# DHDev0/Stochastic-muzero

Hardware: AMD Instinct MI355X
Metric: MCTS simulations/sec (whole node), CartPole MLP 4096 envs × 50 sims (higher is better)
Workload: dtype f32 (tree values, heads) + f64 (pUCT scores, root priors) + i32 (counts)

## Files before the change

### stochastic-muzero_amd/csrc/smz_mlp_device.hpp

```cpp
#pragma once
#include <hip/hip_runtime.h>
#include <math.h>
#include <stdint.h>

#include "../../include/smz.h"

namespace smz_mlp {

constexpr int kWave = 64;
enum { M_DYN_IN, M_ADY_IN, M_DYN_MID, M_ADY_MID, M_DYN_OUT, M_ADY_OUT, M_PRE_IN, M_APR_IN, M_PRE_MID, M_APR_MID,
       M_PRE_OUT, M_APR_OUT, M_REP_IN, M_REP_MID, M_REP_OUT, M_COUNT };

__host__ __device__ inline int up4(int x) { return (x + 3) & ~3; }

typedef float v2f __attribute__((ext_vector_type(2)));
__device__ inline v2f pk_fma(float wx, float wy, float ax, float ay, v2f c) {
    v2f w = {wx, wy}, a = {ax, ay};
    return __builtin_elementwise_fma(w, a, c);
}
template <int U, int R, bool SAME = false>
__device__ inline void dense(const float *const (&W)[R], const float *const (&bias)[R], const float *const (&act)[R], int K4,
                             const int (&OP)[R], int lane, float (&acc)[R][U]) {
    const float4 *a4[R], *w4[R];
    v2f acc2[R][U];
// ... 515 lines not shown

constexpr int kRows = 1;

__host__ __device__ inline int row_scratch_floats(const smz_mlp_desc &d) {
    const int kin = up4(d.S + d.A) > up4(d.obs) ? up4(d.S + d.A) : up4(d.obs);
    return kin + up4(d.H) + up4(d.S);
}
__host__ __device__ inline int scratch_floats(const smz_mlp_desc &d) { return kRows * row_scratch_floats(d); }

template <int U, int R, bool SAME = false, bool CP = false>
__device__ inline void recurrent_rows(const float *lds, const smz_mlp_desc &d, float *scratch, const float *const (&xin)[R],
                                      const bool (&dyn)[R], const bool (&live)[R], float *const (&dst_hidden)[R],
                                      float *const (&dst_policy)[R], float (&reward)[R], float (&value)[R]) {
    const int S = d.S, A = d.A, K4in = up4(S + A), K4h = up4(d.H), K4s = up4(S);
    const int lane = threadIdx.x & (kWave - 1);
    const int rs = row_scratch_floats(d), kin = rs - K4h - K4s;
    float *tA[R], *hbuf[R];
    MatOff m1[R], m1m[R], m3[R], m3m[R];
#pragma unroll
    for (int r = 0; r < R; r++) {
        tA[r] = scratch + r * rs + kin;
        hbuf[r] = tA[r] + K4h;
        m1[r] = pick<CP>(d, dyn[r], M_DYN_IN, M_ADY_IN);   m1m[r] = pick<CP>(d, dyn[r], M_DYN_MID, M_ADY_MID);
        m3[r] = pick<CP>(d, dyn[r], M_PRE_IN, M_APR_IN);   m3m[r] = pick<CP>(d, dyn[r], M_PRE_MID, M_APR_MID);
        for (int k = lane; k < K4s; k += kWave) hbuf[r][k] = 0.f;
    }
    trunk<U, R, SAME>(lds, d, m1, m1m, xin, K4in, tA, lane);
    float acc[R][U];
    constexpr bool PAIRED = SMZ_PAIR_TAILS && U == 1 && R == 2;
    const bool halves = PAIRED && SAME && SMZ_DENSE_HALVES && S <= 32 && !dyn[0] && !dyn[1];
    if (halves) {
        if constexpr (PAIRED && SAME) {
            const MatOff m = pick<CP>(d, false, M_DYN_OUT, M_ADY_OUT);
            acc[0][0] = dense_halves(lds + m.w, lds + m.b, tA[0], tA[1], K4h, m.op, lane);
            acc[1][0] = 0.f;
        }
    } else {
        const float *W[R], *Bv[R], *Ac[R];
        int op[R];
#pragma unroll
        for (int r = 0; r < R; r++) {
            const MatOff m = pick<CP>(d, dyn[r], M_DYN_OUT, M_ADY_OUT);
            W[r] = lds + m.w; Bv[r] = lds + m.b; Ac[r] = tA[r]; op[r] = m.op;
        }
        dense<U, R, SAME>(W, Bv, Ac, K4h, op, lane, acc);
    }
    float pair_rnum = 0.f, pair_rden = 0.f;
    bool pair_reward = false;
    if constexpr (PAIRED) {
        if (S <= 32) {
            reward[0] = reward[1] = 0.f;
            if (halves) scale_pair<true>(acc[0][0], 0.f, S, lane, hbuf[0], hbuf[1], live[0] ? dst_hidden[0] : nullptr,
                                         live[1] ? dst_hidden[1] : nullptr);
            else if (!dyn[0] && !dyn[1]) scale_pair(acc[0][0], acc[1][0], S, lane, hbuf[0], hbuf[1], live[0] ? dst_hidden[0] : nullptr,
                                               live[1] ? dst_hidden[1] : nullptr);
            else if (SMZ_ONE_DECODE) {
                dynamics_tail_pair<true>(acc[0][0], acc[1][0], dyn[0], dyn[1], S, lane, hbuf[0], hbuf[1], live[0] ? dst_hidden[0] : nullptr,
                                         live[1] ? dst_hidden[1] : nullptr, reward[0], reward[1], &pair_rnum, &pair_rden);
                pair_reward = true;
            } else dynamics_tail_pair(acc[0][0], acc[1][0], dyn[0], dyn[1], S, lane, hbuf[0], hbuf[1], live[0] ? dst_hidden[0] : nullptr,
                                      live[1] ? dst_hidden[1] : nullptr, reward[0], reward[1]);
        } else {
#pragma unroll
            for (int r = 0; r < R; r++) {
                reward[r] = 0.f;
                if (dyn[r]) reward[r] = decode_scale_lanes<U>(acc[r], S, lane, hbuf[r], live[r] ? dst_hidden[r] : nullptr);
                else scale_lanes<U>(acc[r], 0, S, lane, hbuf[r], live[r] ? dst_hidden[r] : nullptr);
            }
        }
    } else {
#pragma unroll
    for (int r = 0; r < R; r++) {
        reward[r] = 0.f;
        if (dyn[r]) {
            reward[r] = decode_scale_lanes<U>(acc[r], S, lane, hbuf[r], live[r] ? dst_hidden[r] : nullptr);
        } else {
            scale_lanes<U>(acc[r], 0, S, lane, hbuf[r], live[r] ? dst_hidden[r] : nullptr);
        }
    }
    }
    lds_sync();
    {
        const float *Hc[R];
#pragma unroll
        for (int r = 0; r < R; r++) Hc[r] = hbuf[r];
        trunk<U, R, SAME>(lds, d, m3, m3m, Hc, K4s, tA, lane);
        const float *W[R], *Bv[R], *Ac[R];
        int op[R];
#pragma unroll
        for (int r = 0; r < R; r++) {
            const MatOff m = pick<CP>(d, dyn[r], M_PRE_OUT, M_APR_OUT);
            W[r] = lds + m.w; Bv[r] = lds + m.b; Ac[r] = tA[r]; op[r] = m.op;
        }
        dense<U, R, SAME>(W, Bv, Ac, K4h, op, lane, acc);
    }
    if constexpr (PAIRED) {
        if (S <= 32 && A <= 32 && pair_reward) {
            float r0, r1;
            softmax_decode_pair<true>(acc[0][0], acc[1][0], A, S, lane, live[0] ? dst_policy[0] : nullptr,
                                      live[1] ? dst_policy[1] : nullptr, value[0], value[1], pair_rnum, pair_rden, &r0, &r1);
            reward[0] = dyn[0] ? r0 : 0.f;
            reward[1] = dyn[1] ? r1 : 0.f;
        } else if (S <= 32 && A <= 32) {
            softmax_decode_pair(acc[0][0], acc[1][0], A, S, lane, live[0] ? dst_policy[0] : nullptr, live[1] ? dst_policy[1] : nullptr,
                                value[0], value[1]);
        } else {
#pragma unroll
            for (int r = 0; r < R; r++) value[r] = softmax_decode_lanes<U>(acc[r], A, S, lane, live[r] ? dst_policy[r] : nullptr);
        }
    } else {
#pragma unroll
    for (int r = 0; r < R; r++) {
        value[r] = softmax_decode_lanes<U>(acc[r], A, S, lane, live[r] ? dst_policy[r] : nullptr);
    }
    }
    lds_sync();
}

template <int U, bool CP = false>
__device__ inline void initial_row(const float *lds, const smz_mlp_desc &d, const float *rep, const smz_mlp_desc &drep,
                                   float *scratch, const float *obs_row, float *dst_hidden0, float *dst_hidden1,
                                   float *dst_policy) {
    const int S = d.S, A = d.A, K4o = up4(d.obs), K4h = up4(d.H), K4s = up4(S);
    const int lane = threadIdx.x & (kWave - 1);
    const int rs = row_scratch_floats(d), kin = rs - K4h - K4s;
    float *xbuf = scratch;
    float *tA[1] = {scratch + kin};
    float *hbuf = tA[0] + K4h;
    for (int k = lane; k < K4o; k += kWave) xbuf[k] = (k < d.obs) ? obs_row[k] : 0.f;
    for (int k = lane; k < K4s; k += kWave) hbuf[k] = 0.f;
    lds_sync();
    const MatOff mi[1] = {pick(drep, true, M_REP_IN, M_REP_IN)}, mm[1] = {pick(drep, true, M_REP_MID, M_REP_MID)};
    const float *xi[1] = {xbuf};
    trunk<U, 1>(rep, drep, mi, mm, xi, K4o, tA, lane);
    float acc[1][U];
    {
        const float *W[1] = {rep + drep.off[M_REP_OUT]}, *Bv[1] = {rep + drep.off[M_COUNT + M_REP_OUT]}, *Ac[1] = {tA[0]};
        dense<U, 1>(W, Bv, Ac, K4h, d.OP, lane, acc);
    }
    scale_lanes<U>(acc[0], 0, S, lane, hbuf, dst_hidden0, dst_hidden1);
    lds_sync();
    const MatOff pi[1] = {pick<CP>(d, true, M_PRE_IN, M_PRE_IN)}, pm[1] = {pick<CP>(d, true, M_PRE_MID, M_PRE_MID)};
    const float *hi[1] = {hbuf};
    trunk<U, 1>(lds, d, pi, pm, hi, K4s, tA, lane);
    {
        const MatOff po = pick<CP>(d, true, M_PRE_OUT, M_PRE_OUT);
        const float *W[1] = {lds + po.w}, *Bv[1] = {lds + po.b}, *Ac[1] = {tA[0]};
        dense<U, 1>(W, Bv, Ac, K4h, po.op, lane, acc);
    }
    softmax_lanes<U>(acc[0], A, lane, dst_policy);
    lds_sync();
}

__host__ __device__ inline int rep_floats(const smz_mlp_desc &d) { return d.off[M_COUNT] - d.off[M_REP_IN]; }
__host__ __device__ inline smz_mlp_desc lds_desc_without_rep(const smz_mlp_desc &d) {
    smz_mlp_desc l = d;
    const int rs = rep_floats(d);
    for (int m = 0; m < M_COUNT; m++) l.off[M_COUNT + m] = d.off[M_COUNT + m] - rs;
    l.total_floats = d.total_floats - rs;
    return l;
}
__device__ inline void stage_weights_without_rep(float *lds, const float *weights, const smz_mlp_desc &d) {
    constexpr int UB = 8;
    const int n_mat = d.off[M_REP_IN], n_bias = d.total_floats - d.off[M_COUNT], rs = rep_floats(d);
    for (int pass = 0; pass < 2; pass++) {
        const float *src = pass ? weights + d.off[M_COUNT] : weights;
        float *dst = pass ? lds + d.off[M_COUNT] - rs : lds;
        const int cnt = pass ? n_bias : n_mat;
        for (int i0 = threadIdx.x * 4; i0 < cnt; i0 += blockDim.x * 4 * UB) {
            float4 v[UB];
#pragma unroll
            for (int u = 0; u < UB; u++) { const int i = i0 + u * blockDim.x * 4; v[u] = *reinterpret_cast<const float4 *>(src + (i < cnt ? i : i0)); }
#pragma unroll
            for (int u = 0; u < UB; u++) { const int i = i0 + u * blockDim.x * 4; if (i < cnt) *reinterpret_cast<float4 *>(dst + i) = v[u]; }
        }
    }
    __syncthreads();
}

__host__ __device__ inline int compact_matrix_floats(const smz_mlp_desc &d) { return mat_off<true>(d, M_REP_IN); }
__host__ __device__ inline int compact_total_floats(const smz_mlp_desc &d) { return compact_matrix_floats(d) + (d.total_floats - d.off[M_COUNT]); }
__device__ inline smz_mlp_desc lds_desc_compact(const smz_mlp_desc &d) {
    smz_mlp_desc l = d;
    l.off[M_COUNT] = compact_matrix_floats(d);
    l.total_floats = compact_total_floats(d);
    return l;
}
__device__ inline void stage_weights_compact(float *lds, const float *weights, const smz_mlp_desc &d) {
    const int kin = up4(d.S + d.A), kmid = d.L > 0 ? up4(d.H) : 0, kh = up4(d.H), ks = up4(d.S);
    const int K[M_REP_IN] = {kin, kin, kmid, kmid, kh, kh, ks, ks, kmid, kmid, kh, kh};
    int dst = 0;
#pragma unroll
    for (int m = 0; m < M_REP_IN; m++) {
        const int op = mat_op<true>(d, m), groups = K[m] >> 2, per = op;
        const float4 *src = reinterpret_cast<const float4 *>(weights + d.off[m]);
        float4 *out = reinterpret_cast<float4 *>(lds + dst);
        for (int i = threadIdx.x; i < groups * per; i += blockDim.x) {
            const int g = i / per, o = i - g * per;
            out[i] = src[g * d.OP + o];
        }
        dst += K[m] * op;
    }
    const int n_bias = d.total_floats - d.off[M_COUNT];
    for (int i = threadIdx.x * 4; i < n_bias; i += blockDim.x * 4)
        *reinterpret_cast<float4 *>(lds + dst + i) = *reinterpret_cast<const float4 *>(weights + d.off[M_COUNT] + i);
    __syncthreads();
}

__device__ inline void stage_recurrent_weights(float *lds, const float *weights, const smz_mlp_desc &d) {
    const int ranges[4] = {0, d.off[M_REP_IN], d.off[M_COUNT], d.off[M_COUNT + M_REP_IN] - d.off[M_COUNT]};
    stage_weights(lds, weights, ranges, 2);
}
__device__ inline void stage_all_weights(float *lds, const float *weights, const smz_mlp_desc &d) {
    const int ranges[2] = {0, d.total_floats};
    stage_weights(lds, weights, ranges, 1);
}
__device__ inline void stage_initial_weights(float *lds, const float *weights, const smz_mlp_desc &d) {
    const int ranges[10] = {d.off[M_REP_IN], d.off[M_COUNT] - d.off[M_REP_IN],
                            d.off[M_PRE_IN], d.off[M_APR_IN] - d.off[M_PRE_IN],
                            d.off[M_PRE_MID], d.off[M_APR_MID] - d.off[M_PRE_MID],
                            d.off[M_PRE_OUT], d.off[M_APR_OUT] - d.off[M_PRE_OUT],
                            d.off[M_COUNT], d.total_floats - d.off[M_COUNT]};
    stage_weights(lds, weights, ranges, 5);
}

}
```

### stochastic-muzero_amd/csrc/smz_search_mlp.hpp

```cpp
#pragma once
#include "smz_common.hpp"
#include "smz_handle.hpp"

namespace {

extern __shared__ float4 smz_search_lds4[];

#ifndef SMZ_BPS_HBM
#define SMZ_BPS_HBM 1
#endif
#ifndef SMZ_SELECT_BLOCKS
#define SMZ_SELECT_BLOCKS 1
#endif
#ifndef SMZ_EARLY_ROWS
#define SMZ_EARLY_ROWS 1
#endif
#ifndef SMZ_PAIR_A4
#define SMZ_PAIR_A4 1
#endif
#ifndef SMZ_SELECT_TWO_PASSES
#define SMZ_SELECT_TWO_PASSES 1
#endif
#ifndef SMZ_LEAF_FIRST
#define SMZ_LEAF_FIRST 1
#endif
#ifndef SMZ_EARLY_STAGE
#define SMZ_EARLY_STAGE 1
#endif
#ifndef SMZ_SELECT_MASKS
#define SMZ_SELECT_MASKS 1
#endif
#ifdef SMZ_BPS_PROBE
#define SMZ_PROBE_DECL unsigned long long pb_t0 = 0, pb_acc[7] = {0, 0, 0, 0, 0, 0, 0};
#define SMZ_PROBE_START pb_t0 = __builtin_amdgcn_s_memtime();
#define SMZ_PROBE_AT(i) { const unsigned long long pb_t1 = __builtin_amdgcn_s_memtime(); pb_acc[i] += pb_t1 - pb_t0; pb_t0 = pb_t1; }
#if SMZ_BPS_PROBE + 0 == 2
#define SMZ_PROBE(i)
#define SMZ_PROBE_B(i) SMZ_PROBE_AT(i)
#else
#define SMZ_PROBE(i) SMZ_PROBE_AT(i)
#define SMZ_PROBE_B(i)
#endif
#define SMZ_PROBE_FLUSH(stats) if ((stats) && lane == 0) { for (int pb_i = 0; pb_i < 7; pb_i++) atomicAdd(&(stats)[8 + pb_i], pb_acc[pb_i]); }
#else
#define SMZ_PROBE_DECL
#define SMZ_PROBE_START
#define SMZ_PROBE(i)
#define SMZ_PROBE_B(i)
#define SMZ_PROBE_FLUSH(stats)
#endif

struct MegaLds {
    int pbc_off, wave_off, per_wave;
    int x_off, pv_off, rng_off, out_off, sel_off, sel_n;
    int sel_on;
    int trees_off, tree_words;
};
__host__ __device__ inline MegaLds mega_lds(const smz_mlp_desc &d, const Params &P, int tpw, bool tlds = false, int waves = 8) {
    MegaLds m;
    m.pbc_off = r4(tlds ? smz_mlp::compact_total_floats(d) : d.total_floats - smz_mlp::rep_floats(d));
    m.wave_off = m.pbc_off + r4(2 * 2 * (P.sims + 2));
    m.x_off = r4(2 * smz_mlp::row_scratch_floats(d));
    m.pv_off = m.x_off + tpw * smz_mlp::up4(P.S + P.A);
    m.rng_off = m.pv_off + tpw * P.P * 4;
    m.out_off = m.rng_off + r4(tpw * kRngStride);
    m.sel_off = m.out_off + r4(tpw * (P.A + 2));
    m.sel_n = (P.sims + 2 + 1) & ~1;
    bool sel = tlds;
    if (!tlds && SMZ_BPS_HBM && P.A == 2 && P.K == 2 && tpw == 2 && P.sims <= 126) {
        const int per = m.sel_off + r4(tpw * m.sel_n);
        sel = ((size_t)m.wave_off + (size_t)waves * per) * sizeof(float) <= (size_t)160 * 1024;
    }
    m.sel_on = sel ? 1 : 0;
    m.per_wave = m.sel_off + (sel ? r4(tpw * m.sel_n) : 0);
    m.tree_words = r4(P.rb_words + P.sims * 6 * P.K + (P.K == 2 ? 2 * P.sims : 0));
    m.trees_off = m.wave_off + waves * m.per_wave;
    return m;
}

constexpr int kFastTpw = 2, kFastS = 31, kFastH = 64, kFastL = 0;
template <int MAXA, int KS, int U, bool INSTR, bool AEX, bool MSK = true, bool PHX = false, bool TLDS = false>
__global__ void __launch_bounds__(SMZ_SEARCH_THREADS) k_search_mlp(Params Pin, smz_mlp_desc d, const float *weights, const float *obs,
                                                    int train, ActOut act, EnvStep env) {
    Params P = Pin;
    P.tree0 = 0;
    if (AEX) { P.A = MAXA; P.tpw = kFastTpw; d.A = MAXA; d.S = kFastS; d.H = kFastH; d.L = kFastL; d.OP = smz_mlp::kWave; P.S = kFastS; }
    if (AEX) P.philox = PHX ? 1 : 0;
    if (KS > 0) P.K = KS;
    fix_layout(P, AEX, KS > 0);
    if (AEX) P.hs = (kFastS + 15) & ~15;
    float *lds = reinterpret_cast<float *>(smz_search_lds4);
    static_assert(!TLDS || (AEX && KS > 0), "LDS-resident trees: the specialised instantiations only");
    const smz_mlp_desc dl = TLDS ? smz_mlp::lds_desc_compact(d) : smz_mlp::lds_desc_without_rep(d);
    if (TLDS) smz_mlp::stage_weights_compact(lds, weights, d);
    else smz_mlp::stage_weights_without_rep(lds, weights, d);
    const int lane = threadIdx.x & (kWave - 1), wave = threadIdx.x / kWave, waves = blockDim.x / kWave;
    const int A = P.A, S = P.S, tpw = P.tpw;
    const MegaLds ml = mega_lds(d, P, tpw, TLDS, waves);
    uint32_t *const nodes_global = P.nodes;
    const int gl_eb_words = P.eb_words;
    if (TLDS) {
        uint32_t *nodes_lds = reinterpret_cast<uint32_t *>(lds + ml.trees_off);
        for (int i = threadIdx.x; i < waves * tpw * ml.tree_words; i += blockDim.x) nodes_lds[i] = 0u;
        P.nodes = nodes_lds;
        P.tree0 = blockIdx.x * waves * tpw;
        P.eb_words = 6 * KS;
        P.tree_words = ml.tree_words;
    }
    constexpr bool THR = AEX && KS == 2, YV = THR && TLDS;
    if (THR) {
        P.thr_off = TLDS ? P.rb_words + P.sims * 6 * KS : P.rb_words + 12;
        P.thr_stride = TLDS ? 2 : P.eb_words;
        P.ry_off = (YV && MAXA <= 8 && P.rp_off + 3 * A <= P.rb_words) ? P.rp_off + 2 * A : -1;
    }
    double *pbc_lds = reinterpret_cast<double *>(lds + ml.pbc_off);
    const int n_pbc = P.sims + 2;
    for (int i = threadIdx.x; i < n_pbc; i += blockDim.x) {
        pbc_lds[i] = P.pbc_sqrt[i];
        pbc_lds[n_pbc + i] = i > 0 ? 1.0 / (double)i : 0.0;
    }
    const int slot = A + 2;
    const int K4in = smz_mlp::up4(S + A);
    float *scratch = lds + ml.wave_off + wave * ml.per_wave;
    float *xall = scratch + ml.x_off;
    uint4 *pvals = reinterpret_cast<uint4 *>(scratch + ml.pv_off);
    uint32_t *rng_tile = reinterpret_cast<uint32_t *>(scratch + ml.rng_off);
    float *outs = scratch + ml.out_off;
    __syncthreads();

    const int tree0 = (blockIdx.x * waves + wave) * tpw;
    const int tree = tree0 + lane;
    const bool valid = lane < tpw && tree < P.B && (!MSK || tree_active(P, tree));
    if (MSK && __ballot(valid) == 0ull) {
        if (env.state && lane < tpw && tree < P.B) cartpole_env_step(env, tree, P.B, act.action, act.policy, act.child_visits, act.root_value);
        return;
    }

    for (int t = 0; t < tpw; t++) {
        const int row = tree0 + t;
        if (row >= P.B) break;
        if (MSK && !__shfl((int)valid, t)) continue;
        smz_mlp::initial_row<U, TLDS>(lds, dl, weights, d, scratch, obs + (size_t)row * d.obs, P.hidden + (size_t)row * P.N * P.hs,
                                      nullptr, outs + t * slot);
    }
    constexpr bool PHC = !AEX || PHX;
    int packed = wave_stage_rng<PHC>(P, tree, valid, rng_tile);
    RngT<PHC> rng;
    rng.bind(P, tree, valid);
    TreeHdr h = {0, 0, 0.f, 0.f, 0, 0.f, 0, 0};
    if (valid) {
        rng.load(P.mt + (size_t)tree * kMtN, packed, rng_tile + lane * kRngStride, kRngStage);
        root_init_tree<MAXA>(P, tree, rng, outs + lane * slot, nullptr, train != 0);
        h = P.hdr[tree];
        packed = rng.pack();
    }
    unsigned n_dec = 0, n_chance = 0, n_children = 0, n_desc = 0;
    const int vmask = MSK ? __builtin_amdgcn_readlane((int)valid, 0) | (__builtin_amdgcn_readlane((int)valid, 1) << 1) : 3;
#define SMZ_SLOT_VALID(src) (MSK ? ((vmask >> (src)) & 1) != 0 : tree0 + (src) < P.B)
    const bool prof = INSTR && (P.dbg & 16) && P.stats;
    const int dbg = INSTR ? P.dbg : 0;
    unsigned long long t_stage = 0, t_expand = 0, t_select = 0, t_mlp = 0, t0 = 0, t1 = 0;
#define SMZ_STAMP(acc) if (INSTR && prof) { t1 = __builtin_amdgcn_s_memtime(); acc += t1 - t0; t0 = t1; }
    constexpr int SU = 2;
    const bool split = P.tpw <= SU;
    if (P.sims > 0 && !(dbg & 8)) packed = wave_stage_rng_from<4, PHC>(P, tree, valid, rng_tile, packed, rng.block());
    uint32_t lin0 = 0u, lin1 = 0u;
    uint64_t anc0 = 0ull, anc1l = 0ull, anc1h = 0ull;
    SMZ_PROBE_DECL
    for (int s = 0; s < P.sims; s++) {
        if (INSTR && prof) t0 = __builtin_amdgcn_s_memtime();
        SMZ_PROBE_START
        Leaf L = {0, 0, 0, 0};
        __builtin_amdgcn_s_setprio(SMZ_PRIO_TREE);
        constexpr bool LBKP = AEX && !INSTR;
        float leaf_rw = 0.f;
        if (valid) {
            rng.load(P.mt + (size_t)tree * kMtN, packed, rng_tile + lane * kRngStride, kRngStage);
            if (s > 0 && !(dbg & 4)) expand_backup_tree<MAXA, KS, LBKP, THR, YV>(P, tree, rng, h, outs + lane * slot, outs[lane * slot + A + 1],
                                                      outs[lane * slot + A], pvals + lane * P.P, &leaf_rw);
        }
        SMZ_PROBE_B(0)
        if constexpr (LBKP) {
            if (s > 0) {
                const int src = lane & (kFastTpw - 1);
                const int len = pick_lane01(h.path_len, src);
                const float lrw = pick_lane01(leaf_rw, src);
                if (lane < 8 * kFastTpw && SMZ_SLOT_VALID(src)) {
                    const bool own = lane < kFastTpw;
                    float mn = own ? h.mn : __builtin_inff(), mx = own ? h.mx : -__builtin_inff(), v_root = 0.f;
                    backup_levels_lanes<kFastTpw, YV>(P, tree0 + src, lane / kFastTpw, len, outs[src * slot + A], lrw,
                                                  pvals + src * P.P, mn, mx, v_root);
                    if (own) {
                        const float nvs = h.root_value_sum + v_root;
                        const int nvc = h.root_visit + 1;
                        h.root_value_sum = nvs;
                        h.root_visit = nvc;
                        const float qv = nvs / (float)nvc;
                        if (qv > mx) mx = qv;
                        if (qv < mn) mn = qv;
                        h.mn = mn;
                        h.mx = mx;
                    }
                }
            }
        }
        SMZ_STAMP(t_expand)
        SMZ_PROBE(0)
        SMZ_PROBE_B(1)
        constexpr bool PAIR = AEX && (MAXA == 2 || (SMZ_PAIR_A4 && MAXA == 4)) && (KS == 2 || (SMZ_PAIR_K4 && KS == 4 && MAXA == 4)) && !INSTR;
        constexpr bool BPS = SMZ_SELECT_BLOCKS && AEX && KS == 2 && (TLDS || SMZ_BPS_HBM) && !INSTR && MAXA == 2;
        bool bps_done = false;
        bool bps_all = false;
        float early_row[kFastTpw] = {0.f, 0.f};
        StagePre<SU> pre;
        bool staged_early = false;
        auto descent_words = [&](int len) {
            const int nw = select_words(len, A);
            rng.used += nw; rng.ready -= nw; rng.idx += nw;
            if (rng.idx >= kMtN) { rng.idx -= kMtN; rng.wrapped(); }
            packed = rng.pack();
        };
        auto early_requests = [&](int len, auto parent_node) {
#if SMZ_EARLY_ROWS
            bps_all = __ballot(valid && len == 0) == 0ull && __ballot(valid) != 0ull;
#if SMZ_EARLY_STAGE
            if (valid && len > 0) descent_words(len);
#endif
            if (bps_all) {
                int par = 0;
                if (valid && len > 1) par = parent_node();
                __builtin_amdgcn_fence(__ATOMIC_SEQ_CST, "workgroup");
#pragma unroll
                for (int t = 0; t < kFastTpw; t++) {
                    const int parent = __builtin_amdgcn_readlane(par, t);
                    const float *srow = P.hidden + ((size_t)(tree0 + t) * P.N + parent) * P.hs;
                    early_row[t] = (lane < S && tree0 + t < P.B) ? srow[lane] : 0.f;
                }
#if SMZ_EARLY_STAGE
                if (split && !(dbg & 8)) { stage_issue<SU, PHC>(P, tree, valid, packed, pre); staged_early = true; }
#endif
            }
#endif
        };
        constexpr bool MASKS = SMZ_SELECT_MASKS && BPS && TLDS;
        const bool masks_on = MASKS && P.sims <= smz_masks::kMaxBlocks;
        if constexpr (MASKS) if (masks_on) {
            namespace mk = smz_masks;
            if (s > 0) {
                int hand = 0;
                if (valid) {
                    const int loc = (int)pvals[lane * P.P + h.path_len - 1].x;
                    hand = h.n_exp | (loc & 0x7f00) | ((loc & 1) << 16) | (h.path_len << 17);
                }
#pragma unroll
                for (int t = 0; t < kFastTpw; t++) {
                    if (!SMZ_SLOT_VALID(t)) continue;
                    const int hw = __builtin_amdgcn_readlane(hand, t);
                    const int e = hw & 255, pb = (hw >> 8) & 255, pl = mk::lane_of(pb, t);
                    const uint64_t q0 = readlane64(anc0, pl), q1l = readlane64(anc1l, pl), q1h = readlane64(anc1h, pl);
                    uint64_t a0, a1;
                    mk::anc_child(pb < 32 ? q0 : q1l, pb < 32 ? 0ull : q1h, pb, t, a0, a1);
                    const uint32_t lin = mk::lin_pack(hw >> 17, pb, (hw >> 16) & 1);
                    if (lane == mk::lane_of(e, t)) {
                        if (e < 32) { lin0 = lin; anc0 = a0; }
                        else { lin1 = lin; anc1l = a0; anc1h = a1; }
                    }
                }
            }
            smz_mlp::lds_sync();
            const int src = lane & 1;
            const int nexp = pick_lane01(valid ? h.n_exp : -1, src), rvis = pick_lane01(h.root_visit, src);
            const float bmn = pick_lane01(h.mn, src), bmx = pick_lane01(h.mx, src);
            const int bused = pick_lane01(valid ? rng.used : 0, src), bstaged = pick_lane01(valid ? rng.staged : 0, src);
            const int bstage = pick_lane01(valid ? (int)(rng.stage - rng_tile) : 0, src);
            const int nmax = max(__builtin_amdgcn_readlane(valid ? h.n_exp : -1, 0), __builtin_amdgcn_readlane(valid ? h.n_exp : -1, 1));
            const uint32_t *stb = tree_base(P, tree0 + src);
            SMZ_PROBE(1)
            uint32_t r0 = 0u, rv0 = 0u, rs0 = 0u, rw0 = 0u, r1 = 0u, rv1 = 0u, rs1 = 0u, rw1 = 0u;
            for (int p = 0; p * (kWave / 2) <= nmax; p++) {
                const int b = p * (kWave / 2) + (lane >> 1);
                uint32_t r = 0u, rv = 0u, rs = 0u, rw = 0u;
                if (b <= nexp) {
                    Kids<2> k;
                    r = select_block_kids<MAXA, YV, RngT<PHC>>(P, stb, b, mk::lin_depth(p ? lin1 : lin0), rvis, bmn, bmx, rng_tile + bstage, bused,
                                                               bstaged, pbc_lds, k);
                    if (r) {
                        const bool pk = (r & 0x80u) != 0u;
                        rv = (uint32_t)(pk ? k.vis[1] : k.vis[0]);
                        rs = __float_as_uint(pk ? k.vsum[1] : k.vsum[0]);
                        rw = __float_as_uint(pk ? k.rew[1] : k.rew[0]);
                        r |= (uint32_t)(b == 0 ? (int)pk : (pk ? k.act[1] : k.act[0])) << 9;
                    }
                }
                if (p == 0) { r0 = r; rv0 = rv; rs0 = rs; rw0 = rw; }
                else { r1 = r; rv1 = rv; rs1 = rs; rw1 = rw; }
            }
            SMZ_PROBE(2)
            const int b0 = lane >> 1, b1 = kWave / 2 + (lane >> 1);
            const uint64_t p0 = __ballot((r0 & 0x80u) != 0u), p1 = __ballot((r1 & 0x80u) != 0u);
            const bool gd0 = b0 <= nexp && mk::good(b0, lin0, src, p0, p1), gd1 = b1 <= nexp && mk::good(b1, lin1, src, p0, p1);
            const uint64_t g0 = __ballot(gd0), g1 = __ballot(gd1);
            const bool on0 = mk::on_path(gd0, anc0, 0ull, g0, g1), on1 = mk::on_path(gd1, anc1l, anc1h, g0, g1);
            const bool ok0 = (r0 & 0x100u) != 0u, ok1 = (r1 & 0x100u) != 0u;
            const uint64_t fb = __ballot((on0 && !ok0) || (on1 && !ok1));
            const bool lf0 = on0 && ok0 && (r0 & 127u) == 0u, lf1 = on1 && ok1 && (r1 & 127u) == 0u;
            const uint64_t lf = __ballot(lf0 || lf1);
            const uint32_t mine = lf0 ? mk::leaf_pack(b0, lin0, (r0 >> 7) & 1u, (r0 >> 9) & 1u, A) : mk::leaf_pack(b1, lin1, (r1 >> 7) & 1u, (r1 >> 9) & 1u, A);
            uint32_t lw = 0u;
#pragma unroll
            for (int t = 0; t < kFastTpw; t++) {
                const int ll = mk::leaf_lane(lf, t);
                if ((fb & mk::tree_lanes(t)) == 0ull && ll >= 0) {
                    const uint32_t w = (uint32_t)__builtin_amdgcn_readlane((int)mine, ll);
                    if (lane == t) lw = w;
                }
            }
            const int len = valid ? mk::leaf_len(lw) : 0;
            SMZ_PROBE(3)
            early_requests(len, [&] { return mk::leaf_parent(lw); });
            if ((fb & mk::tree_lanes(src)) == 0ull) {
                if (on0) pvals[src * P.P + mk::lin_depth(lin0)] = make_uint4((uint32_t)(b0 << 8) | ((r0 >> 7) & 1u), rv0, rs0, rw0);
                if (on1) pvals[src * P.P + mk::lin_depth(lin1)] = make_uint4((uint32_t)(b1 << 8) | ((r1 >> 7) & 1u), rv1, rs1, rw1);
            }
            if (valid && len > 0) {
                const int loc = mk::leaf_loc(lw);
                L.leaf_id = mk::child_node(loc >> 8, loc & 1, A);
                L.parent_id = len > 1 ? mk::leaf_parent(lw) : 0;
                L.action = mk::leaf_action(lw);
                L.branch = depth_flag(len - 1);
#if !(SMZ_EARLY_ROWS && SMZ_EARLY_STAGE)
                descent_words(len);
#endif
                h.path_len = len;
                bps_done = true;
            }
        }
        if constexpr (BPS) if (!masks_on && (TLDS || ml.sel_on)) {
            uint16_t *selw = reinterpret_cast<uint16_t *>(scratch + ml.sel_off);
            const int SELN = ml.sel_n;
            if (valid && s > 0) selw[lane * SELN + h.n_exp] = (uint16_t)(h.path_len << 9);
            smz_mlp::lds_sync();
            const int src = lane & 1;
            const int nexp = pick_lane01(valid ? h.n_exp : -1, src), rvis = pick_lane01(h.root_visit, src);
            const float bmn = pick_lane01(h.mn, src), bmx = pick_lane01(h.mx, src);
            const int bused = pick_lane01(valid ? rng.used : 0, src), bstaged = pick_lane01(valid ? rng.staged : 0, src);
            const int bstage = pick_lane01(valid ? (int)(rng.stage - rng_tile) : 0, src);
            const int nmax = max(__builtin_amdgcn_readlane(valid ? h.n_exp : -1, 0), __builtin_amdgcn_readlane(valid ? h.n_exp : -1, 1));
            const uint32_t *stb = tree_base(P, tree0 + src);
            SMZ_PROBE(1)
            if constexpr (!TLDS && SMZ_SELECT_LOADS_FIRST && SMZ_SELECT_TWO_PASSES) {
                constexpr int NP = SMZ_SELECT_TWO_PASSES > 1 ? SMZ_SELECT_TWO_PASSES : 2;
                for (int base = 0; base <= nmax; base += NP * (kWave / 2)) {
                    BlockRaw raw[NP];
#pragma unroll
                    for (int p = 0; p < NP; p++) {
                        const int b = base + p * (kWave / 2) + (lane >> 1);
                        if (b <= nexp) select_block_request<MAXA, YV>(P, stb, b, raw[p]);
// ... 11 lines not shown
                }
            } else
            for (int base = 0; base <= nmax; base += kWave / 2) {
                const int b = base + (lane >> 1);
                if (b <= nexp) {
                    const int depth = b == 0 ? 0 : (int)(selw[src * SELN + b] >> 9);
                    const uint32_t r = select_block<MAXA, YV, RngT<PHC>, !TLDS>(P, stb, b, depth, rvis, bmn, bmx, rng_tile + bstage, bused, bstaged,
                                                                        pbc_lds);
                    selw[src * SELN + b] = (uint16_t)((depth << 9) | r);
                }
            }
            smz_mlp::lds_sync();
            SMZ_PROBE(2)
            uint16_t *pathw = selw + tpw * SELN;
            int len = 0;
            if (valid) len = select_chase(selw + lane * SELN, pathw + lane * SELN);
            smz_mlp::lds_sync();
            SMZ_PROBE(3)
            const int blen = pick_lane01(len, src);
            early_requests(len, [&] { const int loc = pathw[lane * SELN + len - 2], pb = loc >> 8; return pb == 0 ? 1 + (loc & 3) : 1 + A + (pb - 1) * 2 + (loc & 3); });
            if constexpr (!TLDS && SMZ_LEAF_FIRST) { if (valid && len > 0) L = select_leaf(P, stb, pathw + lane * SELN, len); }
            for (int d = lane >> 1; d < blen; d += kWave / 2) select_record(P, stb, pathw + src * SELN, d, pvals + src * P.P);
            if (valid && len > 0) {
                if constexpr (TLDS || !SMZ_LEAF_FIRST) L = select_leaf(P, stb, pathw + lane * SELN, len);
#if !(SMZ_EARLY_ROWS && SMZ_EARLY_STAGE)
                descent_words(len);
#endif
                h.path_len = len;
                bps_done = true;
            }
        }
        if constexpr (BPS) {
            if (valid && !bps_done) {
                int len = 0;
                L = select_tree<MAXA, KS, false, true, false, THR, YV>(P, tree, rng, h, pbc_lds, len, n_dec, n_chance, n_children, pvals + lane * P.P);
                h.path_len = len;
                packed = rng.pack();
            }
        } else if constexpr (PAIR) {
            const int src = lane & 1;
            const int pk = pick_lane01(valid ? rng.pack() : 0, src), us = pick_lane01(valid ? rng.used : 0, src);

            const float hmn = pick_lane01(h.mn, src), hmx = pick_lane01(h.mx, src);
            const int hrv = pick_lane01(h.root_visit, src);
            const uint32_t pb = (uint32_t)pick_lane01((int)rng.block(), src), pk0 = (uint32_t)pick_lane01((int)rng.key0(), src),
                           pk1 = (uint32_t)pick_lane01((int)rng.key1(), src);
            if (lane < 4 && SMZ_SLOT_VALID(src)) {
                TreeHdr hs = h;
                if (lane >= 2) {
                    rng.load(P.mt + (size_t)(tree0 + src) * kMtN, pk, rng_tile + src * kRngStride, kRngStage);
                    rng.used = us;
                    rng.follow(pb, pk0, pk1);
                    hs.mn = hmn; hs.mx = hmx; hs.root_visit = hrv;
                }
                int len = 0;
                const Leaf Lp = select_tree<MAXA, KS, false, true, true, THR, YV>(P, tree0 + src, rng, hs, pbc_lds, len, n_dec, n_chance,
                                                                             n_children, pvals + src * P.P, lane >> 1);
                if (lane < 2) {
                    L = Lp;
                    h.path_len = len;
                    packed = rng.pack();
                }
            }
        } else if (valid) {
            int len = 0;
            if (dbg & 2) { L.leaf_id = 1; L.parent_id = 0; L.action = 0; L.branch = 0; len = 1; }
            else L = select_tree<MAXA, KS, INSTR, true, false, THR, YV>(P, tree, rng, h, pbc_lds, len, n_dec, n_chance, n_children, pvals + lane * P.P);
            h.path_len = len;
            if (INSTR) n_desc++;
            packed = rng.pack();
        }
        SMZ_STAMP(t_select)
        SMZ_PROBE(4)
        SMZ_PROBE_B(2)
        __builtin_amdgcn_s_setprio(SMZ_PRIO_HEADS);
        if (!(BPS && SMZ_EARLY_ROWS && bps_all)) __builtin_amdgcn_fence(__ATOMIC_SEQ_CST, "workgroup");
        if (split && !(dbg & 8) && !staged_early) stage_issue<SU, PHC>(P, tree, valid, packed, pre);
        if (BPS && SMZ_EARLY_ROWS && bps_all) {
#pragma unroll
            for (int t = 0; t < kFastTpw; t++) {
                if (tree0 + t >= P.B) break;
                const int act = __builtin_amdgcn_readlane(L.action, t);
                if (lane < K4in) xall[t * K4in + lane] = (lane < S) ? early_row[t] : ((lane < S + A && (lane - S) == act) ? 1.f : 0.f);
            }
        } else
        for (int t = 0; t < tpw; t++) {
            const int row = tree0 + t;
            if (row >= P.B) break;
            const int parent = __builtin_amdgcn_readlane(L.parent_id, t), act = __builtin_amdgcn_readlane(L.action, t);
            const float *src = P.hidden + ((size_t)row * P.N + parent) * P.hs;
            for (int k = lane; k < K4in; k += kWave)
                xall[t * K4in + k] = (k < S) ? src[k] : ((k < S + A && (k - S) == act) ? 1.f : 0.f);
        }
        smz_mlp::lds_sync();
        SMZ_PROBE_B(3)
        bool paired = false;
        if (tpw == 2 && !(dbg & 1)) {
            const int b0 = __builtin_amdgcn_readlane(L.branch, 0), b1 = __builtin_amdgcn_readlane(L.branch, 1);
            if (tree0 + 1 < P.B) {
                const float *xin[2] = {xall, xall + K4in};
                const bool dyn[2] = {b0 != 0, b1 != 0};
                float *dh[2], *dp[2] = {outs, outs + slot};
                float reward[2], value[2];
#pragma unroll
                for (int r = 0; r < 2; r++)
                    dh[r] = P.hidden + ((size_t)(tree0 + r) * P.N + __builtin_amdgcn_readlane(L.leaf_id, r)) * P.hs;
                const bool live[2] = {MSK ? (vmask & 1) != 0 : true, MSK ? (vmask & 2) != 0 : true};
                if (b0 == b1) smz_mlp::recurrent_rows<U, 2, true, TLDS>(lds, dl, scratch, xin, dyn, live, dh, dp, reward, value);
                else smz_mlp::recurrent_rows<U, 2, false, TLDS>(lds, dl, scratch, xin, dyn, live, dh, dp, reward, value);
                SMZ_PROBE_B(4)
                if (lane == 0) {
                    outs[A] = value[0]; outs[A + 1] = reward[0];
                    outs[slot + A] = value[1]; outs[slot + A + 1] = reward[1];
                }
                paired = true;
            }
        }
        for (int t = 0; t < tpw && !paired; t += smz_mlp::kRows) {
            if (tree0 + t >= P.B) break;
            constexpr int R = smz_mlp::kRows;
            const float *xin[R];
            bool dyn[R], live[R];
            float *dh[R], *dp[R];
            float reward[R], value[R];
#pragma unroll
            for (int r = 0; r < R; r++) {
                live[r] = (t + r < tpw) && (tree0 + t + r < P.B);
                const int tt = live[r] ? t + r : t;
                live[r] = live[r] && (!MSK || __shfl((int)valid, tt) != 0);
                const int row = tree0 + tt;
                const int leaf = __builtin_amdgcn_readlane(L.leaf_id, tt);
                dyn[r] = __builtin_amdgcn_readlane(L.branch, tt) != 0;
                xin[r] = xall + tt * K4in;
                dh[r] = P.hidden + ((size_t)row * P.N + leaf) * P.hs;
                dp[r] = outs + tt * slot;
            }
            if (!(dbg & 1)) smz_mlp::recurrent_rows<U, R, false, TLDS>(lds, dl, scratch, xin, dyn, live, dh, dp, reward, value);
#pragma unroll
            for (int r = 0; r < R; r++)
                if (live[r] && lane == 0) { outs[(t + r) * slot + A] = value[r]; outs[(t + r) * slot + A + 1] = reward[r]; }
        }
        smz_mlp::lds_sync();
        SMZ_STAMP(t_mlp)
        SMZ_PROBE(5)
        SMZ_PROBE_B(5)
        if (!(dbg & 8)) packed = split ? stage_finish<SU, PHC>(P, tree, valid, rng_tile, packed, pre, rng.block())
                                       : wave_stage_rng_from<4, PHC>(P, tree, valid, rng_tile, packed, rng.block());
        SMZ_STAMP(t_stage)
        SMZ_PROBE(6)
        SMZ_PROBE_B(6)
    }
    SMZ_PROBE_FLUSH(Pin.stats)
#undef SMZ_STAMP
#undef SMZ_SLOT_VALID
    if (INSTR && prof && lane == 0) {
        atomicAdd(&P.stats[4], t_stage); atomicAdd(&P.stats[5], t_expand);
        atomicAdd(&P.stats[6], t_select); atomicAdd(&P.stats[7], t_mlp);
    }
    if (valid) {
        if (P.sims > 0) {
            rng.load(P.mt + (size_t)tree * kMtN, packed, rng_tile + lane * kRngStride, kRngStage);
            expand_backup_tree<MAXA, KS, false, THR, YV>(P, tree, rng, h, outs + lane * slot, outs[lane * slot + A + 1], outs[lane * slot + A],
                                                     pvals + lane * P.P);
            for (int i = 0; i < h.path_len; i++) P.path[(size_t)i * P.B + tree] = pvals[lane * P.P + i];
            packed = rng.pack();
        }
        P.hdr[tree] = h;
        if (act.action) {
            act_tree<MAXA>(P, tree, rng, act.temperature, act.action, act.policy, act.child_visits, act.root_value);
            packed = rng.pack();
        }
        P.rng_pos[tree] = packed;
        rng.save(P, tree);
    }
    if constexpr (TLDS) {
        smz_mlp::lds_sync();
        const int n_blk = 1 + P.sims;
        for (int t = 0; t < tpw; t++) {
            if (tree0 + t >= P.B) break;
            if (MSK && !__shfl((int)valid, t)) continue;
            const uint32_t *src = P.nodes + (size_t)(wave * tpw + t) * P.tree_words;
            uint32_t *dst = nodes_global + (size_t)(tree0 + t) * (P.rb_words + (size_t)P.sims * gl_eb_words);
            for (int i = lane; i < P.rb_words; i += kWave) dst[i] = src[i];
            for (int i = lane; i < (n_blk - 1) * gl_eb_words; i += kWave) {
                const int b = i / gl_eb_words, w = i - b * gl_eb_words;
                dst[P.rb_words + i] = w < P.eb_words ? src[P.rb_words + b * P.eb_words + w] : 0u;
            }
        }
    }
    if (env.state && lane < tpw && tree < P.B)
        cartpole_env_step(env, tree, P.B, act.action, act.policy, act.child_visits, act.root_value);
    if (INSTR) wave_add_stats(P.stats, n_dec, n_chance, n_desc, n_children);
}

}

struct SearchActArgs {
    double temperature;
    int32_t *action;
    double *policy, *child_visits;
    float *root_value;
    EnvStep env;
};

static void name_search_mlp(smz_handle *h, int ks, bool instr, bool aex, bool msk, bool phx, bool tlds) {
    const auto b = [](bool v) { return v ? "true" : "false"; };
    snprintf(h->last_kernel, sizeof(h->last_kernel), "k_search_mlp<%d, %d, 1, %s, %s, %s, %s, %s>", h->maxa, ks, b(instr), b(aex),
             b(msk), b(phx), b(tlds));
}
int smz_internal_search_launch_narrow(smz_handle *h, const smz_mlp_desc *desc, const float *weights_dev, const float *obs_dev,
                                      int train, SearchActArgs a, const double *pow_table_host, smz_stream stream);
int smz_internal_search_launch_wide(smz_handle *h, const smz_mlp_desc *desc, const float *weights_dev, const float *obs_dev,
                                    int train, SearchActArgs a, const double *pow_table_host, smz_stream stream);
int smz_internal_search_launch_tlds(smz_handle *h, const smz_mlp_desc *desc, const float *weights_dev, const float *obs_dev,
                                    int train, SearchActArgs a, Params P, int kWaves, int blocks, size_t lds_t, smz_stream stream);

namespace {

struct SearchLaunch {
    smz_handle *h;
    const smz_mlp_desc *desc;
    const float *weights_dev, *obs_dev;
    int train;
    SearchActArgs a;
    smz_stream stream;
    Params P;
    int kWaves, tpw, blocks, threads;
    size_t lds;
    bool fast;

    int refuse() const {
        if (!h || !desc || !weights_dev || !obs_dev) return fail(SMZ_ERR_INVALID, "smz_search_mlp: null argument%s");
        smz_mlp_desc t = *desc;
        if (smz_mlp_layout(&t) != SMZ_OK || t.total_floats != desc->total_floats)
            return fail(SMZ_ERR_INVALID, "smz_search_mlp: descriptor does not describe an LDS-resident network%s");
        if (desc->A != h->P.A || desc->S != h->P.S)
            return fail(SMZ_ERR_INVALID, "smz_search_mlp: network dimensions differ from the handle's%s");
        return check_dirichlet_alpha(h, train);
    }

    int geometry(const double *pow_table_host) {
        kWaves = 8;
        if (const char *e = getenv("SMZ_SEARCH_WAVES")) { const int v = atoi(e); if ((v == 1 || v == 2 || v == 4 || v == 8 || v == 12 || v == 16) && v * kWave <= SMZ_SEARCH_THREADS) kWaves = v; }
        P = h->P;
        tpw = 1;
        while (tpw < kFastTpw && (size_t)256 * kWaves * tpw < (size_t)P.B) tpw <<= 1;
        if (const char *e = getenv("SMZ_SEARCH_TPW")) { const int v = atoi(e); if (v == 1 || v == 2 || v == 4 || v == 8 || v == 16) tpw = v; }
        P.tpw = tpw;
        const MegaLds ml = mega_lds(*desc, P, tpw, false, kWaves);
        const long long lds_floats = (long long)ml.wave_off + (long long)kWaves * ml.per_wave;
        if (const int rc = check_single_launch_size("smz_search_mlp", tpw, lds_floats)) return rc;
        lds = (size_t)lds_floats * sizeof(float);
        if (a.action && use_pow_table(h, P, a.temperature, pow_table_host, stream) != SMZ_OK) return SMZ_ERR_HIP;
        blocks = (P.B + kWaves * tpw - 1) / (kWaves * tpw);
        threads = kWaves * kWave;
        fast = P.A == h->maxa && tpw == kFastTpw && desc->S == kFastS && desc->H == kFastH && desc->L == kFastL;
        return SMZ_OK;
    }

    ActOut act() const { return ActOut{a.temperature, a.action, a.policy, a.child_visits, a.root_value}; }

    template <int MA, int KS, bool INSTR, bool AEX, bool MSK, bool PHX>
    int launch() const {
        const int rc = launch_with_lds<k_search_mlp<MA, KS, 1, INSTR, AEX, MSK, PHX>>(h, blocks, threads, lds, stream, P, *desc, weights_dev,
                                                                                     obs_dev, train, act(), a.env);
        if (rc == SMZ_OK) name_search_mlp(h, KS, INSTR, AEX, MSK, PHX, false);
        return rc;
    }

    template <class Buckets>
    int launch_buckets() const {
        if (P.stats || P.dbg) return Buckets::template launch<true, false, true, false>(*this);
        if (fast && P.philox) return Buckets::template launch<false, true, true, true>(*this);
        if (fast && !P.active) return Buckets::template launch<false, true, false, false>(*this);
        if (fast) return Buckets::template launch<false, true, true, false>(*this);
        return Buckets::template launch<false, false, true, false>(*this);
    }
};

}
```

Baseline: 539.0 million.

## Batch weight staging with tree zeroing, pair initial rows, lane-parallel final backup

For the LDS-tree fast path with 512-thread blocks, weights are loaded into registers in one batch. The LDS tree zeroing and the pbc table fill run between the loads and the stores, so global latency overlaps with that setup work. The representation and prediction networks for the two trees per wave now run as one paired pass, and RNG stage loads are issued before the initial inference. The final simulation's backup uses the lane-parallel backup helper instead of the serial per-tree one. These changes add template complexity and depend on blockDim being exactly 8 waves for the batch path.

```diff
diff --git a/stochastic-muzero_amd/csrc/smz_mlp_device.hpp b/stochastic-muzero_amd/csrc/smz_mlp_device.hpp
--- a/stochastic-muzero_amd/csrc/smz_mlp_device.hpp
+++ b/stochastic-muzero_amd/csrc/smz_mlp_device.hpp
@@ -691,6 +691,51 @@
     lds_sync();
 }
 
+template <int U, bool CP = false>
+__device__ inline void initial_rows(const float *lds, const smz_mlp_desc &d, const float *rep, const smz_mlp_desc &drep,
+                                    float *scratch, const float *const (&obs_row)[2], float *const (&dst_hidden)[2],
+                                    float *const (&dst_policy)[2]) {
+    static_assert(U == 1, "paired tails: one output per lane");
+    const int S = d.S, A = d.A, K4o = up4(d.obs), K4h = up4(d.H), K4s = up4(S);
+    const int lane = threadIdx.x & (kWave - 1);
+    const int rs = row_scratch_floats(d), kin = rs - K4h - K4s;
+    float *tA[2], *hbuf[2];
+    const float *xi[2], *hi[2];
+#pragma unroll
+    for (int r = 0; r < 2; r++) {
+        float *xbuf = scratch + r * rs;
+        tA[r] = xbuf + kin;
+        hbuf[r] = tA[r] + K4h;
+        xi[r] = xbuf;
+        hi[r] = hbuf[r];
+        for (int k = lane; k < K4o; k += kWave) xbuf[k] = (k < d.obs) ? obs_row[r][k] : 0.f;
+        for (int k = lane; k < K4s; k += kWave) hbuf[r][k] = 0.f;
+    }
+    lds_sync();
+    const MatOff mi = pick(drep, true, M_REP_IN, M_REP_IN), mm = pick(drep, true, M_REP_MID, M_REP_MID);
+    const MatOff mi2[2] = {mi, mi}, mm2[2] = {mm, mm};
+    trunk<U, 2, true>(rep, drep, mi2, mm2, xi, K4o, tA, lane);
+    float acc[2][U];
+    {
+        const float *W[2] = {rep + drep.off[M_REP_OUT], rep + drep.off[M_REP_OUT]};
+        const float *Bv[2] = {rep + drep.off[M_COUNT + M_REP_OUT], rep + drep.off[M_COUNT + M_REP_OUT]}, *Ac[2] = {tA[0], tA[1]};
+        dense<U, 2, true>(W, Bv, Ac, K4h, d.OP, lane, acc);
+    }
+    scale_pair(acc[0][0], acc[1][0], S, lane, hbuf[0], hbuf[1], dst_hidden[0], dst_hidden[1]);
+    lds_sync();
+    const MatOff pi = pick<CP>(d, true, M_PRE_IN, M_PRE_IN), pm = pick<CP>(d, true, M_PRE_MID, M_PRE_MID);
+    const MatOff pi2[2] = {pi, pi}, pm2[2] = {pm, pm};
+    trunk<U, 2, true>(lds, d, pi2, pm2, hi, K4s, tA, lane);
+    {
+        const MatOff po = pick<CP>(d, true, M_PRE_OUT, M_PRE_OUT);
+        const float *W[2] = {lds + po.w, lds + po.w}, *Bv[2] = {lds + po.b, lds + po.b}, *Ac[2] = {tA[0], tA[1]};
+        dense<U, 2, true>(W, Bv, Ac, K4h, po.op, lane, acc);
+    }
+    float v0, v1;
+    softmax_decode_pair(acc[0][0], acc[1][0], A, S, lane, dst_policy[0], dst_policy[1], v0, v1);
+    lds_sync();
+}
+
 __host__ __device__ inline int rep_floats(const smz_mlp_desc &d) { return d.off[M_COUNT] - d.off[M_REP_IN]; }
 __host__ __device__ inline smz_mlp_desc lds_desc_without_rep(const smz_mlp_desc &d) {
     smz_mlp_desc l = d;
@@ -746,6 +791,48 @@
     __syncthreads();
 }
 
+template <int S, int A, int H, int L, int NT, class Between>
+__device__ inline void stage_weights_compact_batch(float *lds, const float *weights, int bias_off, Between &&between) {
+    smz_mlp_desc c = {};
+    c.S = S; c.A = A; c.H = H; c.L = L; c.OP = kWave;
+    constexpr int kin = (S + A + 3) & ~3, kh = (H + 3) & ~3, kmid = L > 0 ? kh : 0, ks = (S + 3) & ~3;
+    const int K[M_REP_IN] = {kin, kin, kmid, kmid, kh, kh, ks, ks, kmid, kmid, kh, kh};
+    constexpr int op_ady = ks < kWave ? ks : kWave, op_pre = ((A + S + 3) & ~3) < kWave ? ((A + S + 3) & ~3) : kWave,
+                  op_dyn = ((2 * S + 3) & ~3) < kWave ? ((2 * S + 3) & ~3) : kWave, op_h = kh < kWave ? kh : kWave;
+    constexpr int n_mat4 = (2 * kin * op_h + 2 * kmid * op_h + kh * op_dyn + kh * op_ady + 2 * ks * op_h + 2 * kmid * op_h + 2 * kh * op_pre) / 4;
+    constexpr int n_bias4 = M_COUNT * kWave / 4, N4 = n_mat4 + n_bias4, NS = (N4 + NT - 1) / NT;
+    typedef float f4 __attribute__((ext_vector_type(4)));
+    const f4 *src4 = reinterpret_cast<const f4 *>(weights);
+    f4 *dst4 = reinterpret_cast<f4 *>(lds);
+    const int tid = threadIdx.x, bias4 = bias_off >> 2;
+    f4 v[NS];
+#pragma unroll
+    for (int k = 0; k < NS; k++) {
+        const int lo_k = k * NT, hi_k = lo_k + NT;
+        int i = lo_k + tid;
+        if (hi_k > N4) i = i < N4 ? i : N4 - 1;
+        int src = bias4 + (i - n_mat4);
+#pragma unroll
+        for (int m = 0; m < M_REP_IN; m++) {
+            const int per = mat_op<true>(c, m), lo = mat_off<true>(c, m) >> 2, hi = lo + (K[m] >> 2) * per;
+            if (hi > lo && hi > lo_k && lo < hi_k) {
+                const int l = i - lo, g = l / per;
+                const int s = (mat_off<false>(c, m) >> 2) + l + (kWave - per) * g;
+                if ((lo <= lo_k || i >= lo) && (hi >= hi_k || i < hi)) src = s;
+            }
+        }
+        v[k] = src4[src];
+    }
+    asm volatile("" ::: "memory");
+    between();
+    asm volatile("" ::: "memory");
+#pragma unroll
+    for (int k = 0; k < NS; k++) {
+        const int i = k * NT + tid;
+        if ((k + 1) * NT <= N4 || i < N4) dst4[i] = v[k];
+    }
+}
+
 __device__ inline void stage_recurrent_weights(float *lds, const float *weights, const smz_mlp_desc &d) {
     const int ranges[4] = {0, d.off[M_REP_IN], d.off[M_COUNT], d.off[M_COUNT + M_REP_IN] - d.off[M_COUNT]};
     stage_weights(lds, weights, ranges, 2);
diff --git a/stochastic-muzero_amd/csrc/smz_search_mlp.hpp b/stochastic-muzero_amd/csrc/smz_search_mlp.hpp
--- a/stochastic-muzero_amd/csrc/smz_search_mlp.hpp
+++ b/stochastic-muzero_amd/csrc/smz_search_mlp.hpp
@@ -92,7 +92,9 @@
     float *lds = reinterpret_cast<float *>(smz_search_lds4);
     static_assert(!TLDS || (AEX && KS > 0), "LDS-resident trees: the specialised instantiations only");
     const smz_mlp_desc dl = TLDS ? smz_mlp::lds_desc_compact(d) : smz_mlp::lds_desc_without_rep(d);
-    if (TLDS) smz_mlp::stage_weights_compact(lds, weights, d);
+    constexpr int kBatchNT = 8 * kWave;
+    const bool batch = TLDS && blockDim.x == kBatchNT;
+    if (TLDS) { if (!batch) smz_mlp::stage_weights_compact(lds, weights, d); }
     else smz_mlp::stage_weights_without_rep(lds, weights, d);
     const int lane = threadIdx.x & (kWave - 1), wave = threadIdx.x / kWave, waves = blockDim.x / kWave;
     const int A = P.A, S = P.S, tpw = P.tpw;
@@ -101,7 +103,7 @@
     const int gl_eb_words = P.eb_words;
     if (TLDS) {
         uint32_t *nodes_lds = reinterpret_cast<uint32_t *>(lds + ml.trees_off);
-        for (int i = threadIdx.x; i < waves * tpw * ml.tree_words; i += blockDim.x) nodes_lds[i] = 0u;
+        if (!batch) for (int i = threadIdx.x; i < waves * tpw * ml.tree_words; i += blockDim.x) nodes_lds[i] = 0u;
         P.nodes = nodes_lds;
         P.tree0 = blockIdx.x * waves * tpw;
         P.eb_words = 6 * KS;
@@ -115,9 +117,25 @@
     }
     double *pbc_lds = reinterpret_cast<double *>(lds + ml.pbc_off);
     const int n_pbc = P.sims + 2;
-    for (int i = threadIdx.x; i < n_pbc; i += blockDim.x) {
+    if (!batch) for (int i = threadIdx.x; i < n_pbc; i += blockDim.x) {
         pbc_lds[i] = P.pbc_sqrt[i];
         pbc_lds[n_pbc + i] = i > 0 ? 1.0 / (double)i : 0.0;
+    }
+    const int tree0 = (blockIdx.x * waves + wave) * tpw;
+    const int tree = tree0 + lane;
+    constexpr bool PHC = !AEX || PHX;
+    constexpr bool ESTG = AEX;
+    int pos_raw = 0;
+    if constexpr (ESTG) pos_raw = P.rng_pos[tree < P.B ? tree : P.B - 1];
+    if constexpr (TLDS) if (batch) {
+        const int ti = threadIdx.x;
+        const double pb = P.pbc_sqrt[ti < n_pbc ? ti : n_pbc - 1];
+        smz_mlp::stage_weights_compact_batch<kFastS, MAXA, kFastH, kFastL, kBatchNT>(lds, weights, d.off[smz_mlp::M_COUNT], [&] {
+            uint4 *z = reinterpret_cast<uint4 *>(P.nodes);
+            for (int i = ti; i < (waves * tpw * ml.tree_words) >> 2; i += kBatchNT) z[i] = make_uint4(0u, 0u, 0u, 0u);
+            if (ti < n_pbc) pbc_lds[n_pbc + ti] = ti > 0 ? 1.0 / (double)ti : 0.0;
+        });
+        if (ti < n_pbc) pbc_lds[ti] = pb;
     }
     const int slot = A + 2;
     const int K4in = smz_mlp::up4(S + A);
@@ -128,23 +146,39 @@
     float *outs = scratch + ml.out_off;
     __syncthreads();
 
-    const int tree0 = (blockIdx.x * waves + wave) * tpw;
-    const int tree = tree0 + lane;
     const bool valid = lane < tpw && tree < P.B && (!MSK || tree_active(P, tree));
     if (MSK && __ballot(valid) == 0ull) {
         if (env.state && lane < tpw && tree < P.B) cartpole_env_step(env, tree, P.B, act.action, act.policy, act.child_visits, act.root_value);
         return;
     }
 
-    for (int t = 0; t < tpw; t++) {
+    int packed = 0;
+    uint32_t block0 = 0u;
+    StagePre<kFastTpw> pre0;
+    if constexpr (ESTG) {
+        packed = valid ? pos_raw : 0;
+        block0 = (PHC && P.philox && valid) ? P.rng_block[tree] : 0u;
+        stage_issue<kFastTpw, PHC>(P, tree, valid, packed, pre0);
+    }
+    bool rooted = false;
+    if constexpr (AEX) {
+        if (tree0 + 1 < P.B && (!MSK || (__builtin_amdgcn_readlane((int)valid, 0) && __builtin_amdgcn_readlane((int)valid, 1)))) {
+            const float *ob[2] = {obs + (size_t)tree0 * d.obs, obs + (size_t)(tree0 + 1) * d.obs};
+            float *dh[2] = {P.hidden + (size_t)tree0 * P.N * P.hs, P.hidden + (size_t)(tree0 + 1) * P.N * P.hs};
+            float *dp[2] = {outs, outs + slot};
+            smz_mlp::initial_rows<U, TLDS>(lds, dl, weights, d, scratch, ob, dh, dp);
+            rooted = true;
+        }
+    }
+    for (int t = 0; t < tpw && !rooted; t++) {
         const int row = tree0 + t;
         if (row >= P.B) break;
         if (MSK && !__shfl((int)valid, t)) continue;
         smz_mlp::initial_row<U, TLDS>(lds, dl, weights, d, scratch, obs + (size_t)row * d.obs, P.hidden + (size_t)row * P.N * P.hs,
                                       nullptr, outs + t * slot);
     }
-    constexpr bool PHC = !AEX || PHX;
-    int packed = wave_stage_rng<PHC>(P, tree, valid, rng_tile);
+    if constexpr (ESTG) packed = stage_finish<kFastTpw, PHC>(P, tree, valid, rng_tile, packed, pre0, block0);
+    else packed = wave_stage_rng<PHC>(P, tree, valid, rng_tile);
     RngT<PHC> rng;
     rng.bind(P, tree, valid);
     TreeHdr h = {0, 0, 0.f, 0.f, 0, 0.f, 0, 0};
@@ -166,6 +200,28 @@
     if (P.sims > 0 && !(dbg & 8)) packed = wave_stage_rng_from<4, PHC>(P, tree, valid, rng_tile, packed, rng.block());
     uint32_t lin0 = 0u, lin1 = 0u;
     uint64_t anc0 = 0ull, anc1l = 0ull, anc1h = 0ull;
+    auto lanes_backup = [&](float leaf_rw) {
+        const int src = lane & (kFastTpw - 1);
+        const int len = pick_lane01(h.path_len, src);
+        const float lrw = pick_lane01(leaf_rw, src);
+        if (lane < 8 * kFastTpw && SMZ_SLOT_VALID(src)) {
+            const bool own = lane < kFastTpw;
+            float mn = own ? h.mn : __builtin_inff(), mx = own ? h.mx : -__builtin_inff(), v_root = 0.f;
+            backup_levels_lanes<kFastTpw, YV>(P, tree0 + src, lane / kFastTpw, len, outs[src * slot + A], lrw,
+                                          pvals + src * P.P, mn, mx, v_root);
+            if (own) {
+                const float nvs = h.root_value_sum + v_root;
+                const int nvc = h.root_visit + 1;
+                h.root_value_sum = nvs;
+                h.root_visit = nvc;
+                const float qv = nvs / (float)nvc;
+                if (qv > mx) mx = qv;
+                if (qv < mn) mn = qv;
+                h.mn = mn;
+                h.mx = mx;
+            }
+        }
+    };
     SMZ_PROBE_DECL
     for (int s = 0; s < P.sims; s++) {
         if (INSTR && prof) t0 = __builtin_amdgcn_s_memtime();
@@ -181,28 +237,7 @@
         }
         SMZ_PROBE_B(0)
         if constexpr (LBKP) {
-            if (s > 0) {
-                const int src = lane & (kFastTpw - 1);
-                const int len = pick_lane01(h.path_len, src);
-                const float lrw = pick_lane01(leaf_rw, src);
-                if (lane < 8 * kFastTpw && SMZ_SLOT_VALID(src)) {
-                    const bool own = lane < kFastTpw;
-                    float mn = own ? h.mn : __builtin_inff(), mx = own ? h.mx : -__builtin_inff(), v_root = 0.f;
-                    backup_levels_lanes<kFastTpw, YV>(P, tree0 + src, lane / kFastTpw, len, outs[src * slot + A], lrw,
-                                                  pvals + src * P.P, mn, mx, v_root);
-                    if (own) {
-                        const float nvs = h.root_value_sum + v_root;
-                        const int nvc = h.root_visit + 1;
-                        h.root_value_sum = nvs;
-                        h.root_visit = nvc;
-                        const float qv = nvs / (float)nvc;
-                        if (qv > mx) mx = qv;
-                        if (qv < mn) mn = qv;
-                        h.mn = mn;
-                        h.mx = mx;
-                    }
-                }
-            }
+            if (s > 0) lanes_backup(leaf_rw);
         }
         SMZ_STAMP(t_expand)
         SMZ_PROBE(0)
@@ -520,16 +555,30 @@
     }
     SMZ_PROBE_FLUSH(Pin.stats)
 #undef SMZ_STAMP
-#undef SMZ_SLOT_VALID
     if (INSTR && prof && lane == 0) {
         atomicAdd(&P.stats[4], t_stage); atomicAdd(&P.stats[5], t_expand);
         atomicAdd(&P.stats[6], t_select); atomicAdd(&P.stats[7], t_mlp);
     }
+    constexpr bool LTAIL = TLDS && AEX && !INSTR;
+    if constexpr (LTAIL) {
+        if (P.sims > 0) {
+            float leaf_rw = 0.f;
+            if (valid) {
+                rng.load(P.mt + (size_t)tree * kMtN, packed, rng_tile + lane * kRngStride, kRngStage);
+                expand_backup_tree<MAXA, KS, true, THR, YV>(P, tree, rng, h, outs + lane * slot, outs[lane * slot + A + 1],
+                                                        outs[lane * slot + A], pvals + lane * P.P, &leaf_rw);
+            }
+            lanes_backup(leaf_rw);
+        }
+    }
+#undef SMZ_SLOT_VALID
     if (valid) {
         if (P.sims > 0) {
-            rng.load(P.mt + (size_t)tree * kMtN, packed, rng_tile + lane * kRngStride, kRngStage);
-            expand_backup_tree<MAXA, KS, false, THR, YV>(P, tree, rng, h, outs + lane * slot, outs[lane * slot + A + 1], outs[lane * slot + A],
-                                                     pvals + lane * P.P);
+            if constexpr (!LTAIL) {
+                rng.load(P.mt + (size_t)tree * kMtN, packed, rng_tile + lane * kRngStride, kRngStage);
+                expand_backup_tree<MAXA, KS, false, THR, YV>(P, tree, rng, h, outs + lane * slot, outs[lane * slot + A + 1],
+                                                         outs[lane * slot + A], pvals + lane * P.P);
+            }
             for (int i = 0; i < h.path_len; i++) P.path[(size_t)i * P.B + tree] = pvals[lane * P.P + i];
             packed = rng.pack();
         }
```

New measurement: 545.8 million (median of 4 runs). 1.01x the previous value.
